# songlab-cal/CherryML

Measured on AMD Instinct MI355X. Metric: cherry-pairs/sec (whole node) per EM iter, higher is better.
Workload: dtype f64

## Files before the change

### cherryml_amd/csrc/eigh_planned.hip.h

```cpp
#pragma once
#include "jacobi_block.hip.h"
#include "large_bank.hip.h"

enum {
  EC_STALL = 0,
  EC_FINAL = 1,
  EC_NSWEEP = 2,
  EC_MODE = 3,
  EC_SQ = 4,
  EC_ERR = 5,
  EC_ARRIVE = 6,
  EC_MASKED = 7,
  EC_SC = 8,
  EC_BANDS = 9,
  EC_SIGMA = 10,
  EC_TBSTALE = 11,
  EC_SKIP = 12,
  EC_REC = 16,
  EC_MAXREC = 12,
  EC_JSTATE = 64,
  EC_T0 = 80,
  EC_TSWEEP = 81,
  EC_TEND = 93,
  EC_NSTAMP = 95,
  EC_STAMPS = 96,
#ifdef CB_EIGH_STAMPS
  EC_WORDS = 96 + 96
#else
  EC_WORDS = 96
#endif
};
#ifdef CB_EIGH_STAMPS
__device__ __forceinline__ void lge_stamp(unsigned long long *ctl, int id) {
  if (blockIdx.x == 0 && blockIdx.y == 0 && threadIdx.x == 0) {
    const unsigned long long i = atomicAdd(ctl + EC_NSTAMP, 1ull);
    if (i < 96ull) ctl[EC_STAMPS + i] = ((unsigned long long)__builtin_amdgcn_s_memrealtime() << 8) | (unsigned long long)id;
  }
}
#define LGE_STAMP(ctl, id) lge_stamp(const_cast<unsigned long long *>(ctl), id)
#else

#define LGE_STAMP(ctl, id) ((void)0)
#endif
#define EC_NONE 0xFFFFFFFFull
#ifdef CB_PLAIN_WORDS
typedef const unsigned long long *lge_const_words;
#else
typedef const __attribute__((address_space(4))) unsigned long long *lge_const_words;
#endif

struct GramArgs {
  int LD, band, slot;
  int cap;
  int nsq;
  const double *G;
  double *X, *Xf;
  double *Gm, *dg;
  int so;
  unsigned long long *acc;
  unsigned long long *ctl;
  double trigger;
};

#define LGE_ACC_NT 32
#define LGE_ACC_COS 64
#define LGE_ACC_WORDS 128
#define LGE_ACC_UNIT 4503599627370496.0
__device__ __forceinline__ unsigned long long lge_fix(double x) {
  return x > 0.0 ? (unsigned long long)(fmin(x, 16.0) * LGE_ACC_UNIT) + 1ull : 0ull;
}

struct DecArgs {
  int on = 0;
  int cap = 0, nsq = 0, so = 0;
  double trigger = 0.0;
  const unsigned long long *acc = nullptr;
};

__device__ __forceinline__ double lge_lim(int order) {
  return order == 2 ? 1e-5 : order == 4 ? 2e-3 : order == 8 ? 0.06 : 0.5;
}

__global__ __launch_bounds__(512, 6) void lge_gram(GramArgs a) {
  __shared__ double sRed[8][256];
  __shared__ double sDg[2][32][16];
  __shared__ double sD[2][16];
  __shared__ double sStat[3][4];
  const unsigned long long *ctl = a.ctl;
  LGE_STAMP(ctl, 4);
  {
    lge_const_words cw = (lge_const_words)ctl;
    const unsigned long long w_stall = cw[EC_STALL], w_final = cw[EC_FINAL];
    if (w_stall != 0ull || (unsigned long long)a.slot > w_final) return;
  }
  const int LD = a.LD, nt = LD / 16;
  const int tm = blockIdx.x / nt, tn = blockIdx.x - tm * nt;
  const int m0 = tm * 16, n0 = tn * 16;
  const int wave = threadIdx.x >> 6, lane = threadIdx.x & 63, lo = lane & 15, hi = lane >> 4;
  const double *rowA = a.G + (size_t)(m0 + lo) * LD + 4 * hi, *rowB = a.G + (size_t)(n0 + lo) * LD + 4 * hi;
  d4 acc0 = {0.0, 0.0, 0.0, 0.0}, acc1 = acc0;
  double da = 0.0, db = 0.0;
  const int nchunks = LD / 16;
  for (int j0 = wave; j0 < nchunks; j0 += 32) {
    d4 av[4], bv[4];
#pragma unroll
    for (int u = 0; u < 4; ++u) {
      const int j = min(j0 + 8 * u, nchunks - 1);
      av[u] = *reinterpret_cast<const d4 *>(rowA + 16 * j);
      bv[u] = *reinterpret_cast<const d4 *>(rowB + 16 * j);
    }
#pragma unroll
    for (int u = 0; u < 4; ++u) {
      if (j0 + 8 * u < nchunks) {
        acc0 = mfma_f64(av[u][0], bv[u][0], acc0);
        acc1 = mfma_f64(av[u][1], bv[u][1], acc1);
        acc0 = mfma_f64(av[u][2], bv[u][2], acc0);
        acc1 = mfma_f64(av[u][3], bv[u][3], acc1);
        da += (av[u][0] * av[u][0] + av[u][1] * av[u][1]) + (av[u][2] * av[u][2] + av[u][3] * av[u][3]);
        db += (bv[u][0] * bv[u][0] + bv[u][1] * bv[u][1]) + (bv[u][2] * bv[u][2] + bv[u][3] * bv[u][3]);
      }
    }
  }
  const d4 acc = acc0 + acc1;
#pragma unroll
  for (int r = 0; r < 4; ++r) sRed[wave][r * 64 + lane] = acc[r];
  sDg[0][wave * 4 + hi][lo] = da;
  sDg[1][wave * 4 + hi][lo] = db;
  __syncthreads();
  if (threadIdx.x < 32) {
    const int w = threadIdx.x >> 4, c = threadIdx.x & 15;
    double s0 = 0.0, s1 = 0.0, s2 = 0.0, s3 = 0.0;
#pragma unroll
    for (int p = 0; p < 32; p += 4) {
      s0 += sDg[w][p][c];
      s1 += sDg[w][p + 1][c];
      s2 += sDg[w][p + 2][c];
      s3 += sDg[w][p + 3][c];
    }
    sD[w][c] = (s0 + s1) + (s2 + s3);
  }
  __syncthreads();
  double mc2 = 0.0;
  if (threadIdx.x < 256) {
    const int t = threadIdx.x, r = t >> 6, l = t & 63;
    const int ri = (l >> 4) + 4 * r, ci = l & 15;
    const int row = m0 + ri, col = n0 + ci;
    double g = 0.0;
#pragma unroll
    for (int w = 0; w < 8; ++w) g += sRed[w][t];
    const double gii = sD[0][ri], gjj = sD[1][ci];
    double x = 0.0;
    const double g2 = g * g, ab = gii * gjj;
    if (!(g2 == g2) || !(ab == ab)) mc2 = INFINITY;
    if (row != col && g2 > ab * (CB_JAC_SKIP * CB_JAC_SKIP)) {
      mc2 = fmax(mc2, g2 * fast_rcp(ab));
      const double d = gjj - gii;
      x = d != 0.0 ? 0.5 * atan(2.0 * g * fast_rcp(d)) : (g > 0.0 ? 0.78539816339744831 : -0.78539816339744831);
    }
    const int bd = row / JB_W - col / JB_W;
    const bool far = bd > a.band || -bd > a.band;
    a.X[(size_t)row * LD + col] = x;
    a.Xf[(size_t)row * LD + col] = far ? x : 0.0;
    if (a.so) {
      a.Gm[(size_t)row * LD + col] = g;
      if (row == col) a.dg[row] = gii;
    }
    double rs = fabs(x), rsf = far ? fabs(x) : 0.0;
#pragma unroll
    for (int m = 1; m < 16; m <<= 1) {
      rs += __shfl_xor(rs, m);
      rsf += __shfl_xor(rsf, m);
      mc2 = fmax(mc2, __shfl_xor(mc2, m));
    }
#pragma unroll
    for (int m = 16; m < 64; m <<= 1) {
      rs = fmax(rs, __shfl_xor(rs, m));
      rsf = fmax(rsf, __shfl_xor(rsf, m));
      mc2 = fmax(mc2, __shfl_xor(mc2, m));
    }
    if (l == 0) {
      sStat[0][r] = rs;
      sStat[1][r] = rsf;
      sStat[2][r] = mc2;
    }
  }
  __syncthreads();
  if (threadIdx.x < 3) {
    const int k = threadIdx.x;
    const double v = fmax(fmax(sStat[k][0], sStat[k][1]), fmax(sStat[k][2], sStat[k][3]));
    if (k < 2) atomicAdd(a.acc + k * LGE_ACC_NT + tm, lge_fix(v));
    else atomicMax(a.acc + LGE_ACC_COS + 16 * (blockIdx.x & 3), dbl_bits(v));
  }
}

struct LgeDecision {
  unsigned long long mode, sq, sc_bits;
};
struct LgeAcc {
  unsigned long long w = 0ull, c2 = 0ull;
};
__device__ __forceinline__ LgeAcc lge_acc_request(const DecArgs &d) {
  LgeAcc q;
  if (d.on) {
    q.w = d.acc[threadIdx.x & 63];
    lge_const_words ar = (lge_const_words)d.acc;
#pragma unroll
    for (int i = 0; i < 4; ++i) {
      const unsigned long long c = ar[LGE_ACC_COS + 16 * i];
      q.c2 = c > q.c2 ? c : q.c2;
    }
  }
  return q;
}
__device__ __forceinline__ double lge_uniform(double v, int lane) {
  return __hiloint2double(__builtin_amdgcn_readlane(__double2hiint(v), lane), __builtin_amdgcn_readlane(__double2loint(v), lane));
}
__device__ __forceinline__ LgeDecision lge_decide_here(int slot, const DecArgs &d, const LgeAcc &q, unsigned long long *ctl,
                                                       unsigned long long nsweep) {
  double v = (double)q.w * (1.0 / LGE_ACC_UNIT);
#pragma unroll
  for (int m = 1; m < 32; m <<= 1) v = fmax(v, __shfl_xor(v, m));
  const double rowsum = lge_uniform(v, 0), rowsum_far = lge_uniform(v, 32);
  double c2;
  memcpy(&c2, &q.c2, 8);
  LgeDecision o{0ull, 0ull, 0x3FF0000000000000ull};
  const bool bad = q.c2 >= 0x7FF0000000000000ull;
  bool masked = false, fin = false;
  if (!bad) {
    masked = c2 > d.trigger * d.trigger || rowsum > 1.0;
    const double rsu = masked ? rowsum_far : rowsum;
    const bool so = d.so != 0 && !masked && c2 > 1e-16 && rowsum <= 0.3;
    const double r2 = rowsum * rowsum;
    fin = !masked && (c2 <= 1e-16 || (so && c2 * r2 * r2 <= 4e-28));
    int order = rsu <= lge_lim(2) ? 2 : rsu <= lge_lim(4) ? 4 : rsu <= lge_lim(8) ? 8 : 12;
    if (order > d.cap) order = d.cap;
    const double lim = lge_lim(order);
    double sc = 1.0;
    while (rsu * sc > lim) {
      sc *= 0.5;
      ++o.sq;
    }
    unsigned long long damped = 0ull;
    if (o.sq > (unsigned long long)d.nsq) {
// ... 45 lines not shown
    double r = -lam[k] * Ut[(size_t)k * LD + i];
    for (int j = 0; j < LD; ++j) r = fma(A[(size_t)i * LD + j], Ut[(size_t)k * LD + j], r);
    m = fmax(m, fabs(r));
    if (!(r == r)) m = INFINITY;
  }
  m = wave_max(m);
  if ((threadIdx.x & 63) == 0) atomicMax(ctl + 92, dbl_bits(m));
}
#endif
#ifdef CB_NANCHECK
__global__ void lge_orthcheck(int LD, const double *R, unsigned long long slot, unsigned long long *ctl) {
  lge_const_words cw = (lge_const_words)ctl;
  if (cw[EC_STALL] != 0ull || slot > cw[EC_FINAL] || !(cw[EC_MODE] >> 16)) return;
  const int k = blockIdx.x;
  double m = 0.0;
  for (int j = threadIdx.x; j < LD; j += blockDim.x) {
    double d = j == k ? -1.0 : 0.0;
    for (int i = 0; i < LD; ++i) d = fma(R[(size_t)i * LD + k], R[(size_t)i * LD + j], d);
    m = fmax(m, fabs(d));
    if (!(d == d)) m = INFINITY;
  }
  m = wave_max(m);
  if ((threadIdx.x & 63) == 0) {
    const unsigned long long old = atomicMax(ctl + 91, dbl_bits(m));
    if (dbl_bits(m) > old) ctl[90] = slot;
  }
}
#endif
#ifdef CB_NANCHECK
__global__ void lge_nancheck(int LD, const double *buf, unsigned long long tag, unsigned long long *ctl) {
  const size_t i = (size_t)blockIdx.x * blockDim.x + threadIdx.x;
  if (i >= (size_t)LD * LD) return;
  const double v = buf[i];
  if (!(v - v == 0.0)) atomicCAS(ctl + 94, 0ull, tag);
}
#endif

enum { EG_P2 = 0, EG_P34, EG_T1, EG_RP, EG_SQ, EG_GR, EG_R4 };

struct EgArgs {
  int LD, slot, kind, q;
  int cap;
  int early;
  const unsigned long long *ctl;
  const double *X, *Xf;
  double *P2, *P4;
  double *B0, *B1, *B2;
  double *T;
  double *R[2], *Rt[2];
  double *Rfin;
  const double *Gin;
  double *Gout;
  DecArgs dec;
  unsigned long long *zacc;
};


__device__ __forceinline__ double lge_ld(const double *base, int s, int LD, int c0, unsigned lane_bytes) {
  const __amdgpu_buffer_rsrc_t rs = __builtin_amdgcn_make_buffer_rsrc(const_cast<double *>(base), 0, 0x7fffffff, 0x00027000);
  return __builtin_bit_cast(double, __builtin_amdgcn_raw_buffer_load_b64(rs, (int)lane_bytes, (int)((unsigned)(4 * s * LD + c0) * 8u), 0));
}

__device__ __forceinline__ double lge_fold8(double (*sRed)[256], d4 acc, int wave, int lane, int et) {
  if (wave >= 4) {
#pragma unroll
    for (int r = 0; r < 4; ++r) sRed[wave - 4][r * 64 + lane] = acc[r];
  }
  __syncthreads();
  if (wave < 4) {
#pragma unroll
    for (int r = 0; r < 4; ++r) acc[r] += sRed[wave][r * 64 + lane];
  }
  __syncthreads();
  if (wave < 4) {
#pragma unroll
    for (int r = 0; r < 4; ++r) sRed[wave][r * 64 + lane] = acc[r];
  }
  __syncthreads();
  return (sRed[0][et] + sRed[1][et]) + (sRed[2][et] + sRed[3][et]);
}

#define LGE_UU 13
template <int KIND>
__global__ __launch_bounds__(512) void lge_gemm(EgArgs a) {
  __shared__ double sRed[4][256];
  const unsigned long long *ctl = a.ctl;
  LGE_STAMP(ctl, 10 + KIND);
  const int LD = a.LD, nt = LD / 16;
  const int tm = blockIdx.x / nt, tn = blockIdx.x - tm * nt;
  const int m0 = tm * 16, n0 = tn * 16;
  const int wave = __builtin_amdgcn_readfirstlane(threadIdx.x >> 6), lane = threadIdx.x & 63, lo = lane & 15, hi = lane >> 4;
  const int nsteps = LD / 4;
  const unsigned loff = (unsigned)(hi * LD + lo) * 8u;
  const int et = threadIdx.x & 255, er = et >> 6, el = et & 63;
  const int row = m0 + (el >> 4) + 4 * er, col = n0 + (el & 15);
  const size_t idx = (size_t)row * LD + col;
  const bool ep = threadIdx.x < 256;
  const double *Ap = nullptr, *Bp = nullptr, *Ep = nullptr;
  if (KIND == EG_T1) { Ap = a.P4; Bp = a.B2; Ep = a.B1; }
  if (KIND == EG_RP) { Ap = a.P4; Bp = a.T; Ep = a.B0; }
  if (KIND == EG_SQ) { Ap = a.Rt[a.q & 1]; Bp = a.R[a.q & 1]; }
  if (KIND == EG_GR) { Ap = a.Rfin; Bp = a.Gin; }
  if (KIND == EG_R4) { Ap = a.P2; Bp = a.B0; Ep = a.P2; }
  double av[LGE_UU], bv[LGE_UU], e1 = 0.0, ex = 0.0;
  const bool early = KIND != EG_P2 && a.early != 0;
  if (early) {
#pragma unroll
    for (int u = 0; u < LGE_UU; ++u) {
      const int sk = min(wave + 8 * u, nsteps - 1);
      av[u] = lge_ld(Ap, sk, LD, m0, loff);
      bv[u] = lge_ld(Bp, sk, LD, n0, loff);
    }
    if (Ep && ep) e1 = Ep[idx];
  }
  LgeAcc accq;
  if (KIND == EG_P2) accq = lge_acc_request(a.dec);
  lge_const_words cw = (lge_const_words)ctl;
  const unsigned long long w_stall = cw[EC_STALL], w_final = cw[EC_FINAL], w_nsw = cw[EC_NSWEEP];
  unsigned long long mode = cw[EC_MODE], w_sq = cw[EC_SQ], w_sc = cw[EC_SC];
  if (w_stall != 0ull || (unsigned long long)a.slot > w_final) return;
  if (KIND == EG_P2 && a.dec.on) {
    const LgeDecision dd = lge_decide_here(a.slot, a.dec, accq, const_cast<unsigned long long *>(ctl), w_nsw);
    mode = dd.mode;
    w_sq = dd.sq;
    w_sc = dd.sc_bits;
  }
  if (!(mode >> 16)) return;
  if (KIND == EG_GR && a.zacc && blockIdx.x == 0 && threadIdx.x < LGE_ACC_WORDS)
    a.zacc[threadIdx.x] = 0ull;
  const int order = (int)(mode & 255ull);
  const bool masked = (mode & (256ull | 1024ull)) != 0ull;
  const int sq = (int)w_sq;
  double sc;
  memcpy(&sc, &w_sc, 8);
  const double *Xu = masked ? a.Xf : a.X;
  if (KIND == EG_R4 && order != 4) return;
  if (KIND == EG_T1 && order != 12) return;
  if (KIND == EG_RP && order < 8) return;
  if (KIND == EG_SQ && a.q >= sq) return;
  if (!early) {
    const double *pa = KIND == EG_P2 ? Xu : Ap, *pb = KIND == EG_P2 ? Xu : Bp;
#pragma unroll
    for (int u = 0; u < LGE_UU; ++u) {
      const int sk = min(wave + 8 * u, nsteps - 1);
      av[u] = lge_ld(pa, sk, LD, m0, loff);
      bv[u] = lge_ld(pb, sk, LD, n0, loff);
    }
    if (KIND != EG_P2 && Ep && ep) e1 = Ep[idx];
  }
  if ((KIND == EG_P2 || KIND == EG_R4) && ep) ex = Xu[idx];
  d4 acc = {0.0, 0.0, 0.0, 0.0};
#pragma unroll
  for (int u = 0; u < LGE_UU; ++u)
    if (wave + 8 * u < nsteps) acc = mfma_f64(av[u], bv[u], acc);
  for (int s0 = wave + 8 * LGE_UU; s0 < nsteps; s0 += 8 * LGE_UU) {
    const double *pa = KIND == EG_P2 ? Xu : Ap, *pb = KIND == EG_P2 ? Xu : Bp;
#pragma unroll
    for (int u = 0; u < LGE_UU; ++u) {
      const int sk = min(s0 + 8 * u, nsteps - 1);
      av[u] = lge_ld(pa, sk, LD, m0, loff);
      bv[u] = lge_ld(pb, sk, LD, n0, loff);
    }
#pragma unroll
    for (int u = 0; u < LGE_UU; ++u)
      if (s0 + 8 * u < nsteps) acc = mfma_f64(av[u], bv[u], acc);
  }
  const double v = lge_fold8(sRed, acc, wave, lane, et);
  if (!ep) return;
  const double edl = row == col ? 1.0 : 0.0, s2 = sc * sc;
  if (KIND == EG_P2) {
    if (order == 2) {
      a.Rfin[idx] = fma(-0.5 * s2, v, fma(sc, ex, edl));
    } else {
      a.P2[idx] = v;
      if (a.cap == 4) a.B0[idx] = fma(-s2 * (1.0 / 24.0), v, (sc * (1.0 / 6.0)) * ex);
    }
  } else if (KIND == EG_R4) {
    a.Rfin[idx] = fma(-s2, v, fma(-0.5 * s2, e1, fma(sc, ex, edl)));
  } else if (KIND == EG_T1) {
    a.T[idx] = fma(s2 * s2, v, e1);
  } else if (KIND == EG_RP) {
    const double o = fma(s2 * s2, v, e1);
    if (sq == 0) a.Rfin[idx] = o;
    else {
      a.R[0][idx] = o;
      a.Rt[0][(size_t)col * LD + row] = o;
    }
  } else if (KIND == EG_SQ) {
    if (a.q == sq - 1) a.Rfin[idx] = v;
    else {
      a.R[(a.q + 1) & 1][idx] = v;
      a.Rt[(a.q + 1) & 1][(size_t)col * LD + row] = v;
    }
  } else {
    a.Gout[idx] = v;
  }
}

__global__ __launch_bounds__(512) void lge_p34(EgArgs a) {
  __shared__ double sRed[8][256];
  const unsigned long long *ctl = a.ctl;
  LGE_STAMP(ctl, 17);
  const int LD = a.LD, nt = LD / 16;
  const int tm = blockIdx.x / nt, tn = blockIdx.x - tm * nt;
  const int m0 = tm * 16, n0 = tn * 16;
  const int wave = __builtin_amdgcn_readfirstlane(threadIdx.x >> 6), lane = threadIdx.x & 63, lo = lane & 15, hi = lane >> 4;
  const int w4 = wave & 3;
  const bool fourth = wave >= 4;
  const int nsteps = LD / 4;
  const unsigned loff = (unsigned)(hi * LD + lo) * 8u;
  const int et = threadIdx.x & 255, er = et >> 6, el = et & 63;
  const int row = m0 + (el >> 4) + 4 * er, col = n0 + (el & 15);
  const size_t idx = (size_t)row * LD + col;
  const bool ep = threadIdx.x < 256;
  double av[LGE_UU], bv[LGE_UU], e2 = 0.0;
  const bool early = a.early != 0;
  if (early) {
#pragma unroll
    for (int u = 0; u < LGE_UU; ++u) {
      const int sk = min(w4 + 4 * u, nsteps - 1);
// ... 24 lines not shown
  } else if (!fourth) {
#pragma unroll
    for (int u = 0; u < LGE_UU; ++u) av[u] = lge_ld(Xu, min(w4 + 4 * u, nsteps - 1), LD, m0, loff);
  }
  double ex = 0.0;
  if (ep) ex = Xu[idx];
  d4 acc = {0.0, 0.0, 0.0, 0.0};
#pragma unroll
  for (int u = 0; u < LGE_UU; ++u)
    if (w4 + 4 * u < nsteps) acc = mfma_f64(av[u], bv[u], acc);
  for (int s0 = w4 + 4 * LGE_UU; s0 < nsteps; s0 += 4 * LGE_UU) {
#pragma unroll
    for (int u = 0; u < LGE_UU; ++u) {
      const int sk = min(s0 + 4 * u, nsteps - 1);
      av[u] = lge_ld(Ap, sk, LD, m0, loff);
      bv[u] = lge_ld(a.P2, sk, LD, n0, loff);
    }
#pragma unroll
    for (int u = 0; u < LGE_UU; ++u)
      if (s0 + 4 * u < nsteps) acc = mfma_f64(av[u], bv[u], acc);
  }
#pragma unroll
  for (int r = 0; r < 4; ++r) sRed[wave][r * 64 + lane] = acc[r];
  __syncthreads();
  if (!ep) return;
  const double p3 = (sRed[0][et] + sRed[1][et]) + (sRed[2][et] + sRed[3][et]);
  const double p4 = (sRed[4][et] + sRed[5][et]) + (sRed[6][et] + sRed[7][et]);
  const double dl = row == col ? 1.0 : 0.0;
  const double s2 = sc * sc;
  const double y1 = sc * ex, y2 = -s2 * e2, y3 = s2 * sc * p3, y4 = s2 * s2 * p4;
  const double b0 = dl + y1 + 0.5 * y2 + y3 * (1.0 / 6.0);
  if (order == 4) {
    a.Rfin[idx] = b0 + y4 * (1.0 / 24.0);
    return;
  }
  a.P4[idx] = p4;
  a.B0[idx] = b0;
  const double b1 = dl * (1.0 / 24.0) + y1 * (1.0 / 120.0) + y2 * (1.0 / 720.0) + y3 * (1.0 / 5040.0);
  if (order == 8) {
    a.T[idx] = b1 + y4 * (1.0 / 40320.0);
    return;
  }
  a.B1[idx] = b1;
  a.B2[idx] = dl * (1.0 / 40320.0) + y1 * (1.0 / 362880.0) + y2 * (1.0 / 3628800.0) + y3 * (1.0 / 39916800.0) + y4 * (1.0 / 479001600.0);
}

struct SoArgs {
  int LD, slot;
  const unsigned long long *ctl;
  const double *Gm, *dg, *X;
  double *Xs;
  int early;
  DecArgs dec;
};

__global__ __launch_bounds__(512) void lge_so(SoArgs a) {
  __shared__ double sRed[4][256];
  const unsigned long long *ctl = a.ctl;
  LGE_STAMP(ctl, 6);
  const int LD = a.LD, nt = LD / 16;
  const int tm = blockIdx.x / nt, tn = blockIdx.x - tm * nt;
  const int m0 = tm * 16, n0 = tn * 16;
  const int wave = threadIdx.x >> 6, lane = threadIdx.x & 63, lo = lane & 15, hi = lane >> 4;
  d4 accA = {0.0, 0.0, 0.0, 0.0}, accB = accA;
  const int nsteps = LD / 4;
  const double *Em = a.Gm + m0 + lo, *En = a.Gm + n0 + lo, *Xm = a.X + m0 + lo, *Xn = a.X + n0 + lo;
  double e1[7], x1[7], x2[7], e2[7];
  auto issue = [&](int s0) {
#pragma unroll
    for (int u = 0; u < 7; ++u) {
      const int s = min(s0 + 8 * u, nsteps - 1);
      const int k = 4 * s + hi;
      const size_t krow = (size_t)k * LD;
      e1[u] = k == m0 + lo ? 0.0 : Em[krow];
      x1[u] = Xn[krow];
      x2[u] = Xm[krow];
      e2[u] = k == n0 + lo ? 0.0 : En[krow];
    }
  };
  if (a.early) issue(wave);
  const LgeAcc accq = lge_acc_request(a.dec);
  lge_const_words cw = (lge_const_words)ctl;
  const unsigned long long w_stall = cw[EC_STALL], w_final = cw[EC_FINAL], w_nsw = cw[EC_NSWEEP];
  unsigned long long w_mode = cw[EC_MODE];
  if (w_stall != 0ull || (unsigned long long)a.slot > w_final) return;
  if (a.dec.on) w_mode = lge_decide_here(a.slot, a.dec, accq, const_cast<unsigned long long *>(ctl), w_nsw).mode;
  if (!(w_mode & 1024ull)) return;
  for (int s0 = wave; s0 < nsteps; s0 += 7 * 8) {
    if (!(a.early && s0 == wave)) issue(s0);
#pragma unroll
    for (int u = 0; u < 7; ++u)
      if (s0 + 8 * u < nsteps) {
        accA = mfma_f64(e1[u], x1[u], accA);
        accB = mfma_f64(x2[u], e2[u], accB);
      }
  }
  d4 acc = accA + accB;
  if (wave >= 4) {
#pragma unroll
    for (int r = 0; r < 4; ++r) sRed[wave - 4][r * 64 + lane] = acc[r];
  }
  __syncthreads();
  if (wave < 4) {
#pragma unroll
    for (int r = 0; r < 4; ++r) acc[r] += sRed[wave][r * 64 + lane];
  }
  __syncthreads();
  if (wave < 4) {
#pragma unroll
    for (int r = 0; r < 4; ++r) sRed[wave][r * 64 + lane] = acc[r];
  }
  __syncthreads();
  if (threadIdx.x >= 256) return;
  const int t = threadIdx.x, r = t >> 6, l = t & 63;
  const int row = m0 + (l >> 4) + 4 * r, col = n0 + (l & 15);
  const double v = (sRed[0][t] + sRed[1][t]) + (sRed[2][t] + sRed[3][t]);
  const size_t idx = (size_t)row * LD + col;
  const double x1v = a.X[idx];
  const double d = a.dg[col] - a.dg[row];
  double xs = x1v;
  if (row != col && x1v != 0.0 && d != 0.0) xs = 0.5 * atan(2.0 * (a.Gm[idx] + 0.5 * v) * fast_rcp(d));
  a.Xs[idx] = xs;
}

__device__ void lge_reset_words(unsigned long long *ctl, unsigned long long *acc) {
  if (threadIdx.x < EC_WORDS)
    ctl[threadIdx.x] = threadIdx.x == EC_FINAL ? EC_NONE : threadIdx.x == EC_T0 ? (unsigned long long)__builtin_amdgcn_s_memrealtime() : 0ull;
  if (threadIdx.x < 2 * LGE_ACC_WORDS) acc[threadIdx.x] = 0ull;
}
__global__ void lge_begin(int LD, const double *A, double *sigma, unsigned long long *ctl, unsigned long long *acc) {
  __shared__ double s[256];
  lge_reset_words(ctl, acc);
  double m = 0.0;
  for (int i = threadIdx.x; i < LD; i += 256) m = fmax(m, fabs(A[(size_t)i * LD + i]));
  s[threadIdx.x] = m;
  __syncthreads();
  for (int st = 128; st >= 1; st >>= 1) {
    if ((int)threadIdx.x < st) s[threadIdx.x] = fmax(s[threadIdx.x], s[threadIdx.x + st]);
    __syncthreads();
  }
  if (threadIdx.x == 0) *sigma = s[0] > 0.0 ? s[0] : 1.0;
}

__global__ __launch_bounds__(512) void lge_plain(int LD, const double *Aop, const double *Bop, const double *Sub, const double *sigma,
                                                 double *out, const unsigned long long *skip) {
  __shared__ double sRed[4][256];
  const int nt = LD / 16;
  const int tm = blockIdx.x / nt, tn = blockIdx.x - tm * nt;
  const int m0 = tm * 16, n0 = tn * 16;
  const int wave = __builtin_amdgcn_readfirstlane(threadIdx.x >> 6), lane = threadIdx.x & 63, lo = lane & 15, hi = lane >> 4;
  const int nsteps = LD / 4;
  const unsigned loff = (unsigned)(hi * LD + lo) * 8u;
  const int et = threadIdx.x & 255, er = et >> 6, el = et & 63;
  const int row = m0 + (el >> 4) + 4 * er, col = n0 + (el & 15);
  const size_t idx = (size_t)row * LD + col;
  double av[LGE_UU], bv[LGE_UU];
#pragma unroll
  for (int u = 0; u < LGE_UU; ++u) {
    const int sk = min(wave + 8 * u, nsteps - 1);
    av[u] = lge_ld(Aop, sk, LD, m0, loff);
    bv[u] = lge_ld(Bop, sk, LD, n0, loff);
  }
  const double e1 = (Sub && threadIdx.x < 256) ? Sub[idx] : 0.0;
  const double sg = sigma ? *sigma : 0.0;
  if (skip && *(lge_const_words)skip != 0ull) return;
  d4 acc = {0.0, 0.0, 0.0, 0.0};
#pragma unroll
  for (int u = 0; u < LGE_UU; ++u)
    if (wave + 8 * u < nsteps) acc = mfma_f64(av[u], bv[u], acc);
// ... 122 lines not shown
```

### cherryml_amd/csrc/eigh_planned_host.hip.h

```cpp
#pragma once

struct EighRecord {
  bool stall = false;
  int err = 0, nsweep = 0, final_slot = -1;
  double sigma = 0.0;
  bool tb_stale = false;
  struct {
    double c, rs, rsf;
    int order, sq, slot;
    bool masked, damped;
  } sweep[EC_MAXREC];
};

#ifndef CB_PLANNED_BAND
#define CB_PLANNED_BAND 1
#endif
#ifndef CB_LEAD_INNER
#define CB_LEAD_INNER 2
#endif
static const int kPlannedBand = CB_PLANNED_BAND;

static void eigh_plan_default(EighPlan &p, int extra = 0) {
  p = EighPlan{};
  p.lead_band = 1;
// ... 62 lines not shown
    memset(q, 0, 2 * (EC_WORDS + 16) * sizeof(unsigned long long));
    h->epin = static_cast<unsigned long long *>(q);
  }
  const int RS = LD + ((2 - LD % 32 + 32) % 32);
  const size_t lds = (size_t)(16 * RS + 3 * 16 * 17 + JB_WAVES * 256) * sizeof(double);
  if (hipFuncSetAttribute(reinterpret_cast<const void *>(lgj_round), hipFuncAttributeMaxDynamicSharedMemorySize, (int)lds) != hipSuccess)
    return false;
  if (hipMemsetAsync(ctl, 0, EC_WORDS * sizeof(unsigned long long), h->stream) != hipSuccess) return false;
  h->ectl = ctl;
  h->planned_unavailable = false;
  return true;
}

#ifdef CB_NANCHECK
#define NANCHECK(buf, tag) hipLaunchKernelGGL(lge_nancheck, dim3((unsigned)((LL + 255) / 256)), dim3(256), 0, h->stream, LD, buf, (unsigned long long)(tag), ctl)
#else
#define NANCHECK(buf, tag) ((void)0)
#endif
static int enqueue_planned_solve(cb_bank *h, const EighPlan &p, unsigned long long seq, int first_slot = 0, double tb_rho_max = 0.0,
                                 const TbTableArgs &tbt = TbTableArgs{}) {
  const int LD = h->LD, nt = LD / 16, nb = LD / JB_W;
  const size_t LL = (size_t)LD * LD;
  unsigned long long *ctl = h->ectl;
  unsigned long long *eacc = reinterpret_cast<unsigned long long *>(h->epart);
  double *Gb[2] = {h->Gc, h->Gc2};
  double *X = h->gx, *Xf = h->gx + LL, *P2 = h->gx + 2 * LL, *P3 = h->gx + 3 * LL, *P4 = h->gx + 4 * LL, *B0 = h->gx + 5 * LL,
         *B1 = h->gx + 6 * LL, *B2 = h->gx + 7 * LL, *T = h->gx + 8 * LL, *R0 = h->gx + 9 * LL, *R0t = h->gx + 10 * LL,
         *R1 = h->gx + 11 * LL, *R1t = h->gx + 6 * LL,
         *Rfin = h->gx + 3 * LL;
  const int RS = LD + ((2 - LD % 32 + 32) % 32);
  const size_t lds = (size_t)(16 * RS + 3 * 16 * 17 + JB_WAVES * 256) * sizeof(double);
  if (first_slot > 0) {
    hipLaunchKernelGGL(lge_resume, dim3(1), dim3(64), 0, h->stream, ctl);
  } else {
    if (!h->begin_folded) hipLaunchKernelGGL(lge_begin, dim3(1), dim3(256), 0, h->stream, LD, h->A, h->sigma, ctl, eacc);
    NANCHECK(h->U, 1);
    NANCHECK(h->A, 2);
    hipLaunchKernelGGL(lge_plain, dim3((unsigned)(nt * nt)), dim3(512), 0, h->stream, LD, h->U, h->A, h->Vc, h->sigma, Gb[0], nullptr);
  }
  unsigned long long *jstate = ctl + EC_JSTATE;
  int shift = 0;
  auto band_pass = [&](double *G, const unsigned long long *must_nonzero) {
    for (int w = 0; w < 2; ++w)
      hipLaunchKernelGGL(lgj_round, dim3(nb / 2), dim3(JB_THREADS), lds, h->stream, LD, ((shift + w) & 1) && nb > 2 ? -2 : -1,
                         must_nonzero ? 1 : CB_LEAD_INNER, G,
                         jstate, ctl + EC_STALL, must_nonzero);
    for (int k = 2; k <= kPlannedBand && k < nb; ++k)
      for (int par = 0; par < 2; ++par)
        hipLaunchKernelGGL(lgj_round, dim3((unsigned)(((nb + 2 * k - 1) / (2 * k)) * k)), dim3(JB_THREADS), lds, h->stream, LD,
                           -(10 + 2 * (k - 2) + par), 0, G, jstate, ctl + EC_STALL, must_nonzero);
    ++shift;
  };
  if (p.lead_band) band_pass(Gb[first_slot & 1], nullptr);
  const dim3 tiles((unsigned)(nt * nt));
  for (int i = 0; i < p.nslots; ++i) {
    const EighSlot &q = p.slot[i];
    const int s = first_slot + i;
    double *Gin = Gb[s & 1], *Gout = Gb[(s + 1) & 1];
    unsigned long long *acc = eacc + (size_t)(s & 1) * LGE_ACC_WORDS;
    GramArgs ga{LD, kPlannedBand, s, q.cap, q.cap == 12 ? q.nsq : 0, Gin, X, Xf, P3, h->epart + (size_t)2 * LGE_ACC_WORDS,
                q.so, acc, ctl, 3e-4};
    NANCHECK(Gin, 1000 + s * 100 + 1);
    hipLaunchKernelGGL(lge_gram, tiles, dim3(512), 0, h->stream, ga);
    NANCHECK(X, 1000 + s * 100 + 2);
    DecArgs dec;
    dec.on = 1; dec.cap = ga.cap; dec.nsq = ga.nsq; dec.so = q.so; dec.acc = acc; dec.trigger = ga.trigger;
#ifdef CB_DECIDE_KERNEL
    hipLaunchKernelGGL(lge_decide_k, dim3(1), dim3(64), 0, h->stream, s, dec, ctl);
    dec.on = 0;
#endif
    if (q.so) {
      SoArgs so{LD, s, ctl, ga.Gm, ga.dg, X, Xf, q.expect_run && i >= 1, dec};
#ifdef CB_NO_EARLY
      so.early = 0;
#endif
      hipLaunchKernelGGL(lge_so, tiles, dim3(512), 0, h->stream, so);
      NANCHECK(Xf, 1000 + s * 100 + 3);
    }
    EgArgs e{};
    if (!q.so) e.dec = dec;
    e.zacc = acc;
    e.LD = LD; e.slot = s; e.cap = q.cap; e.ctl = ctl; e.X = X; e.Xf = Xf; e.P2 = P2; e.P4 = P4; e.B0 = B0; e.B1 = B1; e.B2 = B2; e.T = T;
    e.R[0] = R0; e.R[1] = R1; e.Rt[0] = R0t; e.Rt[1] = R1t; e.Rfin = Rfin; e.Gin = Gin; e.Gout = Gout;
    auto gemm = [&](int kind, int qq = 0) {
      EgArgs c = e;
      c.kind = kind;
      c.q = qq;
      const int xo = q.expect_order;
      c.early = !q.expect_run ? 0 : kind == EG_P34 ? xo >= 4 : kind == EG_T1 ? xo == 12 : kind == EG_RP ? xo >= 8 :
                kind == EG_SQ ? qq < q.expect_sq : kind == EG_R4 ? xo == 4 : 1;
#ifdef CB_NO_EARLY
      c.early = 0;
#endif
      switch (kind) {
        case EG_P2: hipLaunchKernelGGL(lge_gemm<EG_P2>, tiles, dim3(512), 0, h->stream, c); break;
        case EG_P34: hipLaunchKernelGGL(lge_p34, tiles, dim3(512), 0, h->stream, c); break;
        case EG_T1: hipLaunchKernelGGL(lge_gemm<EG_T1>, tiles, dim3(512), 0, h->stream, c); break;
        case EG_RP: hipLaunchKernelGGL(lge_gemm<EG_RP>, tiles, dim3(512), 0, h->stream, c); break;
        case EG_SQ: hipLaunchKernelGGL(lge_gemm<EG_SQ>, tiles, dim3(512), 0, h->stream, c); break;
        case EG_R4: hipLaunchKernelGGL(lge_gemm<EG_R4>, tiles, dim3(512), 0, h->stream, c); break;
        default: hipLaunchKernelGGL(lge_gemm<EG_GR>, tiles, dim3(512), 0, h->stream, c); break;
      }
    };
    gemm(EG_P2);
    if (q.cap == 12) {
      gemm(EG_P34);
      gemm(EG_T1);
      gemm(EG_RP);
      for (int k = 0; k < q.nsq; ++k) gemm(EG_SQ, k);
    } else if (q.cap == 4) {
      gemm(EG_R4);
    }
    NANCHECK(Rfin, 1000 + s * 100 + 4);
#ifdef CB_NANCHECK
    hipLaunchKernelGGL(lge_orthcheck, dim3((unsigned)LD), dim3(256), 0, h->stream, LD, Rfin, (unsigned long long)s, ctl);
#endif
    gemm(EG_GR);
    NANCHECK(Gout, 1000 + s * 100 + 5);
    if (q.band_after) band_pass(Gout, ctl + EC_MASKED);
  }
  volatile unsigned long long *pin = h->epin + (size_t)(seq & 1ull) * (EC_WORDS + 16);
  hipLaunchKernelGGL(lge_norms, dim3((LD + 3) / 4), dim3(256), 0, h->stream, LD, Gb[0], Gb[1], h->X, ctl, pin, seq, h->sigma, tb_rho_max);
  LAUNCH_STOP(stop_event(h, EV_EIGH), lge_finish, dim3((LD + 3) / 4 + 1), dim3(256), 0, h->stream, LD, Gb[0], Gb[1], h->X, h->sigma, h->lam, h->U, h->Vc,
                     ctl, tbt, pin, seq);
#ifdef CB_NANCHECK
  hipLaunchKernelGGL(lge_residual, dim3((unsigned)LD), dim3(256), 0, h->stream, LD, h->A, h->Vc, h->lam, ctl);
#endif
  HIP_TRY(hipGetLastError());
  return CB_OK;
}

static int eigh_planned_record(cb_bank *h, unsigned long long seq, EighRecord &r) {
  volatile unsigned long long *pin = h->epin + (size_t)(seq & 1ull) * (EC_WORDS + 16);
  const auto t0 = std::chrono::steady_clock::now();
  bool got = false;
  for (unsigned it = 0;; ++it) {
    if (pin[EC_WORDS] == seq) {
      got = true;
      break;
    }
    if (it == 0) ++h->record_spins;
#if defined(__x86_64__)
    __builtin_ia32_pause();
#endif
    if ((it & 4095u) == 4095u && std::chrono::duration<double, std::milli>(std::chrono::steady_clock::now() - t0).count() > 200.0) break;
  }
  if (!got) {
    HIP_TRY(hipStreamSynchronize(h->stream));
// ... 70 lines not shown
```

### cherryml_amd/csrc/handle_host.hip.h

```cpp
#pragma once
#include <hip/hip_ext.h>
#include <future>
struct EighSlot {
  int cap = 12;
  int nsq = 0;
  int band_after = 0;
  int so = 0;
  int expect_run = 1, expect_order = 12, expect_sq = 2;
};
struct EighPlan {
  int lead_band = 1;
  int nslots = 0;
  EighSlot slot[EC_MAXREC];
};
struct cb_bank {
  int dev = 0, S = 0, L = 0, B = 0;
  int B_cap = 0;
  hipStream_t xstream[3] = {};
  hipEvent_t ev_fork = nullptr, ev_join[3] = {};
  int tr_epochs = 0;
  uint64_t tr_sig = 0;
  int last_form = 0;
  double tr_pow_b1 = 1.0, tr_pow_b2 = 1.0;
  int dtype = CB_F64;
  int LD = 0;
  bool large = false;
  hipStream_t own_stream = nullptr, stream = nullptr;
  std::vector<void *> allocs;
  std::vector<double> n_host;
  double *t = nullptr;
  double *Ct = nullptr;
  double *n_dev = nullptr;
  double *inv_n = nullptr;
  double *ones = nullptr;
  double *Cq = nullptr;
  int nq = 0;
  double *dirsum = nullptr;
  double *dirsum_g = nullptr;
  int Bl = 0;
  double *t_live = nullptr;
  int *nlive = nullptr;
  std::vector<int> nlive_host;
  double *Q = nullptr, *pi = nullptr, *loss = nullptr, *dQ = nullptr;
  int *status = nullptr;
  double *Gc2 = nullptr, *gx = nullptr;
  int last_light = 0;
  void *comm = nullptr;
  int (*allreduce)(const void *, void *, size_t, int, int, void *, hipStream_t) = nullptr;
  double *inv_n_global = nullptr;
  std::vector<double> n_global;
  bool expm_only = false;
  bool per_bucket_products = false;
  bool sym_counts = false;
  int spec_sweeps = 0;
  double *A = nullptr, *dsq = nullptr, *Gc = nullptr, *Vc = nullptr, *U = nullptr, *lam = nullptr,
         *sigma = nullptr, *F = nullptr, *E = nullptr, *H = nullptr, *Gt = nullptr, *T = nullptr,
         *Mt_part = nullptr, *Mt = nullptr, *X = nullptr, *loss_part = nullptr;
  float *Ct32 = nullptr, *Gt32 = nullptr, *T32 = nullptr, *Uf = nullptr, *Utf = nullptr, *Af = nullptr, *Ff = nullptr;
  unsigned long long *off_bits = nullptr;
  unsigned long long *poll = nullptr;
  unsigned long long poll_seq = 0;
  unsigned long long *ectl = nullptr, *epin = nullptr;
  double *epart = nullptr;
  bool begin_folded = false;
  double *sigma_home = nullptr;
  double *sigma2 = nullptr;
  unsigned long long eseq = 0;
  bool planned_unavailable = false;
  int planned_solves = 0, planned_stalls = 0;
  long long record_spins = 0;
  std::vector<double> epoch_seconds;
  EighPlan eplan;
  int k3_chunk = 0, k3_nchunks = 0;
  double *Yk = nullptr, *Lk = nullptr;
  double phi_delta = 0.0;
  unsigned int *bank_queue = nullptr;
  unsigned char *bank_args = nullptr;
  int bank_slots = 0;
  int bank_claims = 0;
  bool bank_fused = false;
  int bank_kg = 1;
  bool bank_accum = false;
  CbTimeBasisHost tb;
  int tb_set = 0;
  double *tb_Ls[2] = {}, *tb_Lg[2] = {}, *tb_tf[2] = {}, *tb_tg[2] = {};
  std::future<CbTimeBasisHost> tb_next;
  bool tb_next_pending = false;
  int tb_next_epoch = 0;
  size_t tb_ew_lds[4] = {0, 0, 0, 0};
  int tb_builds = 0, tb_stale_epochs = 0;
  bool tb_failed = false;
  bool tb_block = false;
  bool bank_tb = false;
  int last_sweeps = 0;
  double *gn_scratch = nullptr, *gn_partial = nullptr;
  int gn_nw = 0;
  struct {
    double *Qn = nullptr, *QT = nullptr, *colsum = nullptr, *alpha = nullptr, *R = nullptr, *RT = nullptr, *E = nullptr,
           *ET = nullptr, *G = nullptr, *GT = nullptr, *Xbar = nullptr, *lpart = nullptr;
    int *nsq = nullptr;
    int cap_slots = 0;
  } gl;
  std::vector<double> t_host, t_live_host;
  bool have_prev = false;
  double *ws_ptr[16] = {};
  size_t ws_cap[16] = {};
  char *pin = nullptr;
  size_t pin_cap = 0, pin_off = 0;
  bool profile = false;
  int profile_every = 1;
  bool profile_now = false;
  hipEvent_t ev[CB_T_COUNT + 1] = {};
  bool ev_rec[CB_T_COUNT + 1] = {};
  double t_sum[CB_T_COUNT] = {};
  int t_calls = 0;
  bool t_pending = false;
  hipEvent_t ev2[CB_T_COUNT + 1] = {};
  bool ev_rec2[CB_T_COUNT + 1] = {};
  bool t_pending2 = false;
};

// ... 102 lines not shown
```

### cherryml_amd/csrc/train_host.hip.h

```cpp
#pragma once
template <int NW>
static int launch_train_nw(cb_bank *h, const TrainArgs &a) {
  static_assert(NW == 4, "25 .. 32 states: the four-wave form only (see the kernels' launch bounds)");
  const size_t lds = (SmallLds<NW>::TOTAL + 72) * sizeof(double);
  if (h->S <= 24) return fail(CB_EINVAL, "internal: %d states dispatched to the one-kernel trainer", h->S);
  auto kern = small_train_kernel<2, 8, NW>;
  HIP_TRY(hipFuncSetAttribute(reinterpret_cast<const void *>(kern), hipFuncAttributeMaxDynamicSharedMemorySize, (int)lds));
  hipLaunchKernelGGL(kern, dim3(h->L), dim3(NW * 64), lds, h->stream, a);
  HIP_TRY(hipGetLastError());
  return CB_OK;
}

__global__ void tr_stamp(double *out) { *out = (double)__builtin_amdgcn_s_memrealtime(); }

static void set_epoch_seconds(cb_bank *h, const char *ticks, int E, double t_first_s) {
  h->epoch_seconds.assign((size_t)std::max(E, 0), 0.0);
  if (!ticks || E <= 0) return;
  std::vector<double> tk((size_t)E + 1);
  memcpy(tk.data(), ticks, ((size_t)E + 1) * sizeof(double));
  for (int e = 0; e < E; ++e) h->epoch_seconds[e] = t_first_s + (tk[e] - tk[E]) * 1e-8;
}

static int run_fused_training_large(cb_bank *h, double *pi_param, double *up_param, const double *mask, int E,
                                    double lr, int do_adam, int flags, double *loss_curve, double *Q_best,
// ... 52 lines not shown
    return fail(CB_ENOMEM, "fused training: device allocation failed");
  }
  if (dbg) fprintf(stderr, "[cherrybank] large trainer: workspaces ready after %.2f ms\n", now() - t_enter);
  int rc = CB_OK;
#define TRYH(expr) \
  if (rc == CB_OK && (expr) != hipSuccess) rc = fail(CB_EHIP, "%s failed", #expr)
  {
    const size_t up_bytes = (S + nup + SS + 64) * sizeof(double);
    const size_t down_bytes = (S + nup + 2 * (size_t)E + 16 + (2 + (size_t)(d_Qp ? n_pow2 : 0)) * SS + 64) * sizeof(double);
    if (!pin_reserve(h, std::max(up_bytes, down_bytes) + 1024)) {
      release();
      return fail(CB_ENOMEM, "fused training: pinned staging allocation failed");
    }
  }
  if (!resume) {
    TRYH(h2d_staged(h, d_pi, pi_param, S * sizeof(double)));
    TRYH(h2d_staged(h, d_up, up_param, nup * sizeof(double)));
    TRYH(hipMemsetAsync(d_mom, 0, nmom * sizeof(double), h->stream));
    TRYH(hipMemsetAsync(d_Qb, 0, SS * sizeof(double), h->stream));
    TRYH(hipMemsetAsync(d_Ql, 0, SS * sizeof(double), h->stream));
  }
  if (mask && !resume) TRYH(h2d_staged(h, d_mask, mask, SS * sizeof(double)));
  const double init_state[2] = {INFINITY, INFINITY};
  LargeTrain a{};
  a.S = S; a.LD = LD; a.do_adam = do_adam; a.n_pow2 = d_Qp ? n_pow2 : 0;
  a.epoch0 = e0;
  a.p_pi = d_pi; a.p_up = d_up;
  a.m_pi = d_mom; a.v_pi = d_mom + S; a.m_up = d_mom + 2 * (size_t)S; a.v_up = a.m_up + nup;
  a.mask = d_mask; a.lr = lr; a.beta1 = 0.9; a.beta2 = 0.999; a.eps = 1e-8;
  a.pi = d_vec; a.gd = d_vec + LD; a.state = d_vec + LD + S;
  a.dsq = h->dsq; a.A = h->A; a.G = h->Mt; a.loss = h->loss;
  a.dirsum = h->comm ? h->dirsum_g : h->dirsum;
  a.inv_n = (flags & CB_NORMALIZE) ? 1.0 / (h->comm ? h->n_global[0] : h->n_host[0]) : 1.0;
  a.loss_curve = d_loss; a.time_curve = d_time; a.Q_last = d_Ql; a.Q_best = d_Qb; a.Q_pow2 = d_Qp;
  if (dbg) fprintf(stderr, "[cherrybank] large trainer: copies enqueued after %.2f ms\n", now() - t_enter);
  if (!resume) TRYH(h2d_staged(h, a.state, init_state, sizeof init_state));
  TRYH(hipStreamSynchronize(h->stream));
  if (dbg) fprintf(stderr, "[cherrybank] large trainer: synced after %.2f ms\n", now() - t_enter);
  if (h->profile) fold_pending(h);
  if (dbg) fprintf(stderr, "[cherrybank] large trainer: parameters uploaded after %.2f ms\n", now() - t_enter);
  double pow_b1 = resume ? h->tr_pow_b1 : 1.0, pow_b2 = resume ? h->tr_pow_b2 : 1.0;
  if (!h->sigma2) {
    if (dev_alloc(h, &h->sigma2, 2) != CB_OK) {
      release();
      return CB_ENOMEM;
    }
  }
  if (!h->sigma_home) h->sigma_home = h->sigma;
  TRYH(hipMemsetAsync(h->sigma2, 0, 2 * sizeof(double), h->stream));
  h->last_form = 4000;
  h->tr_epochs = 0;
  const int fault_epoch = cb_test_hook("CB_FAULT_INJECT") ? atoi(cb_test_hook("CB_FAULT_INJECT")) : -1000;
  const bool planned = !cb_test_hook("CB_EIGH_HOST") && !cb_test_hook("CB_NO_HYBRID") && LD % 16 == 0 && LD / JB_W >= 8 && eigh_planned_setup(h);
  EighPlan &plan = h->eplan;
  if (!resume) eigh_plan_default(plan);
  if (!resume) {
    tb_drop_next(h);
    h->tb = CbTimeBasisHost{};
    h->tb_failed = false;
  }
  const int short_plans = cb_test_hook("CB_EIGH_SHORT_PLAN") ? std::max(1, atoi(cb_test_hook("CB_EIGH_SHORT_PLAN"))) : 0;
  auto shorten = [&]() {
    if (!short_plans) return;
    plan.nslots = 1;
    if (short_plans >= 2) plan.slot[0] = EighSlot{2, 0, plan.slot[0].band_after, 0};
  };
  shorten();
  const double trace_slow = getenv("CB_TRACE_SLOW") ? atof(getenv("CB_TRACE_SLOW")) : 0.0;
  const double t_first_s = (now() - t_enter) * 1e-3;
  hipLaunchKernelGGL(tr_stamp, dim3(1), dim3(1), 0, h->stream, d_time + E);
  for (int e = 0; e < E && rc == CB_OK; ++e) {
    const double te0 = trace_slow > 0.0 ? now() : 0.0;
    double te_fold = 0.0, te_enq = 0.0, te_rec = 0.0;
    h->profile_now = h->profile && (e0 + e) % h->profile_every == 0;
    if (h->profile_now) {
      swap_event_sets(h);
      fold_pending(h);
    }
    if (trace_slow > 0.0) te_fold = now();
    clear_marks(h);
    const bool use_plan = planned && h->have_prev && e0 + e >= 3;
    {
      const int par = (e0 + e) & 1;
      h->sigma = h->sigma2 + par;
      a.sig_cur = reinterpret_cast<unsigned long long *>(h->sigma2 + par);
      a.sig_next = reinterpret_cast<unsigned long long *>(h->sigma2 + (par ^ 1));
      a.ectl = use_plan ? h->ectl : nullptr;
      a.eacc = use_plan ? reinterpret_cast<unsigned long long *>(h->epart) : nullptr;
      h->begin_folded = use_plan;
    }
    LAUNCH_STOP(stop_event(h, EV_START), lt_build, dim3(LD), dim3(256), 0, h->stream, a, e0 + e);
    rc = large_eval(h, flags & CB_NORMALIZE, h->loss, h->Mt, true, nullptr, false, use_plan ? &plan : nullptr);
    h->begin_folded = false;
    if (trace_slow > 0.0) te_enq = now();
    if (rc == CB_OK && use_plan) {
      EighRecord rec;
      rc = eigh_planned_record(h, h->eseq, rec);
      ++h->planned_solves;
      if (rc == CB_OK && rec.err == 2) rc = fail(CB_ENUMERIC, "eigensolver: non-finite input");
      int slots_done = plan.nslots;
      for (int attempt = 0; rc == CB_OK && rec.stall && attempt < 3; ++attempt) {
        ++h->planned_stalls;
        EighPlan more;
        eigh_plan_continue(rec, more);
        clear_marks(h);
        mark(h, EV_START);
// ... 347 lines not shown
```

Baseline: 1.546 billion.

## Compute only upper-triangle tiles of symmetric Gram/P2/SO products and mirror

The Gram, second-order and P2 GEMM kernels now launch one block per upper-triangular 16x16 tile pair instead of every tile. Each off-diagonal block writes both its tile and the transposed mirror, using the upper 256 threads that were previously idle in the epilogue. A folded index mapping pairs row q with row nt-1-q so blocks stay balanced. This roughly halves the MFMA work and reads for these symmetric products. The cost is extra epilogue stores, per-row accumulator atomics for both rows, and a lower occupancy hint on lge_gram. An env hook restores full tiling.

```diff
diff --git a/cherryml_amd/csrc/eigh_planned.hip.h b/cherryml_amd/csrc/eigh_planned.hip.h
--- a/cherryml_amd/csrc/eigh_planned.hip.h
+++ b/cherryml_amd/csrc/eigh_planned.hip.h
@@ -60,6 +60,7 @@
   unsigned long long *acc;
   unsigned long long *ctl;
   double trigger;
+  int pair;
 };
 
 #define LGE_ACC_NT 32
@@ -81,11 +82,25 @@
   return order == 2 ? 1e-5 : order == 4 ? 2e-3 : order == 8 ? 0.06 : 0.5;
 }
 
-__global__ __launch_bounds__(512, 6) void lge_gram(GramArgs a) {
+__device__ __forceinline__ void lge_tile(int b, int nt, bool pair, int &tm, int &tn) {
+  const int dv = pair ? nt + 1 : nt;
+  const int q = b / dv, c = b - q * dv;
+  tm = q;
+  tn = c;
+  if (pair) {
+    if (c < nt - q) tn = q + c;
+    else {
+      tm = nt - 1 - q;
+      tn = tm + (c - (nt - q));
+    }
+  }
+}
+
+__global__ __launch_bounds__(512, 4) void lge_gram(GramArgs a) {
   __shared__ double sRed[8][256];
   __shared__ double sDg[2][32][16];
   __shared__ double sD[2][16];
-  __shared__ double sStat[3][4];
+  __shared__ double sStat[2][3][4];
   const unsigned long long *ctl = a.ctl;
   LGE_STAMP(ctl, 4);
   {
@@ -94,7 +109,8 @@
     if (w_stall != 0ull || (unsigned long long)a.slot > w_final) return;
   }
   const int LD = a.LD, nt = LD / 16;
-  const int tm = blockIdx.x / nt, tn = blockIdx.x - tm * nt;
+  int tm, tn;
+  lge_tile((int)blockIdx.x, nt, a.pair != 0, tm, tn);
   const int m0 = tm * 16, n0 = tn * 16;
   const int wave = threadIdx.x >> 6, lane = threadIdx.x & 63, lo = lane & 15, hi = lane >> 4;
   const double *rowA = a.G + (size_t)(m0 + lo) * LD + 4 * hi, *rowB = a.G + (size_t)(n0 + lo) * LD + 4 * hi;
@@ -140,15 +156,17 @@
     sD[w][c] = (s0 + s1) + (s2 + s3);
   }
   __syncthreads();
+  const bool mir = threadIdx.x >= 256, two = a.pair != 0 && tm != tn;
   double mc2 = 0.0;
-  if (threadIdx.x < 256) {
-    const int t = threadIdx.x, r = t >> 6, l = t & 63;
+  if (!mir || two) {
+    const int t = threadIdx.x & 255, r = t >> 6, l = t & 63;
     const int ri = (l >> 4) + 4 * r, ci = l & 15;
-    const int row = m0 + ri, col = n0 + ci;
+    const int row = (mir ? n0 : m0) + ri, col = (mir ? m0 : n0) + ci;
+    const int ts = mir ? 16 * ci + ri : t;
     double g = 0.0;
 #pragma unroll
-    for (int w = 0; w < 8; ++w) g += sRed[w][t];
-    const double gii = sD[0][ri], gjj = sD[1][ci];
+    for (int w = 0; w < 8; ++w) g += sRed[w][ts];
+    const double gii = sD[mir ? 1 : 0][ri], gjj = sD[mir ? 0 : 1][ci];
     double x = 0.0;
     const double g2 = g * g, ab = gii * gjj;
     if (!(g2 == g2) || !(ab == ab)) mc2 = INFINITY;
@@ -179,16 +197,16 @@
       mc2 = fmax(mc2, __shfl_xor(mc2, m));
     }
     if (l == 0) {
-      sStat[0][r] = rs;
-      sStat[1][r] = rsf;
-      sStat[2][r] = mc2;
-    }
-  }
-  __syncthreads();
-  if (threadIdx.x < 3) {
-    const int k = threadIdx.x;
-    const double v = fmax(fmax(sStat[k][0], sStat[k][1]), fmax(sStat[k][2], sStat[k][3]));
-    if (k < 2) atomicAdd(a.acc + k * LGE_ACC_NT + tm, lge_fix(v));
+      sStat[mir][0][r] = rs;
+      sStat[mir][1][r] = rsf;
+      sStat[mir][2][r] = mc2;
+    }
+  }
+  __syncthreads();
+  if (threadIdx.x < (two ? 5 : 3)) {
+    const int k = threadIdx.x, h = k >= 3, kk = k - 3 * h;
+    const double v = fmax(fmax(sStat[h][kk][0], sStat[h][kk][1]), fmax(sStat[h][kk][2], sStat[h][kk][3]));
+    if (kk < 2) atomicAdd(a.acc + kk * LGE_ACC_NT + (h ? tn : tm), lge_fix(v));
     else atomicMax(a.acc + LGE_ACC_COS + 16 * (blockIdx.x & 3), dbl_bits(v));
   }
 }
@@ -340,6 +358,7 @@
   const double *Gin;
   double *Gout;
   DecArgs dec;
+  int pair;
   unsigned long long *zacc;
 };
 
@@ -375,15 +394,18 @@
   const unsigned long long *ctl = a.ctl;
   LGE_STAMP(ctl, 10 + KIND);
   const int LD = a.LD, nt = LD / 16;
-  const int tm = blockIdx.x / nt, tn = blockIdx.x - tm * nt;
+  int tm, tn;
+  lge_tile((int)blockIdx.x, nt, KIND == EG_P2 && a.pair != 0, tm, tn);
   const int m0 = tm * 16, n0 = tn * 16;
   const int wave = __builtin_amdgcn_readfirstlane(threadIdx.x >> 6), lane = threadIdx.x & 63, lo = lane & 15, hi = lane >> 4;
   const int nsteps = LD / 4;
   const unsigned loff = (unsigned)(hi * LD + lo) * 8u;
-  const int et = threadIdx.x & 255, er = et >> 6, el = et & 63;
-  const int row = m0 + (el >> 4) + 4 * er, col = n0 + (el & 15);
+  const bool mir = KIND == EG_P2 && a.pair != 0 && tm != tn && threadIdx.x >= 256;
+  const int et = threadIdx.x & 255, eri = et >> 4, eci = et & 15;
+  const int es = mir ? 16 * eci + eri : et;
+  const int row = (mir ? n0 : m0) + eri, col = (mir ? m0 : n0) + eci;
   const size_t idx = (size_t)row * LD + col;
-  const bool ep = threadIdx.x < 256;
+  const bool ep = threadIdx.x < 256 || mir;
   const double *Ap = nullptr, *Bp = nullptr, *Ep = nullptr;
   if (KIND == EG_T1) { Ap = a.P4; Bp = a.B2; Ep = a.B1; }
   if (KIND == EG_RP) { Ap = a.P4; Bp = a.T; Ep = a.B0; }
@@ -453,7 +475,7 @@
     for (int u = 0; u < LGE_UU; ++u)
       if (s0 + 8 * u < nsteps) acc = mfma_f64(av[u], bv[u], acc);
   }
-  const double v = lge_fold8(sRed, acc, wave, lane, et);
+  const double v = lge_fold8(sRed, acc, wave, lane, es);
   if (!ep) return;
   const double edl = row == col ? 1.0 : 0.0, s2 = sc * sc;
   if (KIND == EG_P2) {
@@ -584,6 +606,7 @@
   double *Xs;
   int early;
   DecArgs dec;
+  int pair;
 };
 
 __global__ __launch_bounds__(512) void lge_so(SoArgs a) {
@@ -591,7 +614,8 @@
   const unsigned long long *ctl = a.ctl;
   LGE_STAMP(ctl, 6);
   const int LD = a.LD, nt = LD / 16;
-  const int tm = blockIdx.x / nt, tn = blockIdx.x - tm * nt;
+  int tm, tn;
+  lge_tile((int)blockIdx.x, nt, a.pair != 0, tm, tn);
   const int m0 = tm * 16, n0 = tn * 16;
   const int wave = threadIdx.x >> 6, lane = threadIdx.x & 63, lo = lane & 15, hi = lane >> 4;
   d4 accA = {0.0, 0.0, 0.0, 0.0}, accB = accA;
@@ -643,10 +667,12 @@
     for (int r = 0; r < 4; ++r) sRed[wave][r * 64 + lane] = acc[r];
   }
   __syncthreads();
-  if (threadIdx.x >= 256) return;
-  const int t = threadIdx.x, r = t >> 6, l = t & 63;
-  const int row = m0 + (l >> 4) + 4 * r, col = n0 + (l & 15);
-  const double v = (sRed[0][t] + sRed[1][t]) + (sRed[2][t] + sRed[3][t]);
+  const bool mir = threadIdx.x >= 256;
+  if (mir && !(a.pair != 0 && tm != tn)) return;
+  const int t = threadIdx.x & 255, ri = t >> 4, ci = t & 15;
+  const int ts = mir ? 16 * ci + ri : t;
+  const int row = (mir ? n0 : m0) + ri, col = (mir ? m0 : n0) + ci;
+  const double v = (sRed[0][ts] + sRed[1][ts]) + (sRed[2][ts] + sRed[3][ts]);
   const size_t idx = (size_t)row * LD + col;
   const double x1v = a.X[idx];
   const double d = a.dg[col] - a.dg[row];
diff --git a/cherryml_amd/csrc/eigh_planned_host.hip.h b/cherryml_amd/csrc/eigh_planned_host.hip.h
--- a/cherryml_amd/csrc/eigh_planned_host.hip.h
+++ b/cherryml_amd/csrc/eigh_planned_host.hip.h
@@ -138,16 +138,17 @@
     ++shift;
   };
   if (p.lead_band) band_pass(Gb[first_slot & 1], nullptr);
-  const dim3 tiles((unsigned)(nt * nt));
+  const int pair = h->eigh_full_tiles ? 0 : 1;
+  const dim3 tiles((unsigned)(nt * nt)), mtiles((unsigned)(pair ? nt * (nt + 1) / 2 : nt * nt));
   for (int i = 0; i < p.nslots; ++i) {
     const EighSlot &q = p.slot[i];
     const int s = first_slot + i;
     double *Gin = Gb[s & 1], *Gout = Gb[(s + 1) & 1];
     unsigned long long *acc = eacc + (size_t)(s & 1) * LGE_ACC_WORDS;
     GramArgs ga{LD, kPlannedBand, s, q.cap, q.cap == 12 ? q.nsq : 0, Gin, X, Xf, P3, h->epart + (size_t)2 * LGE_ACC_WORDS,
-                q.so, acc, ctl, 3e-4};
+                q.so, acc, ctl, 3e-4, pair};
     NANCHECK(Gin, 1000 + s * 100 + 1);
-    hipLaunchKernelGGL(lge_gram, tiles, dim3(512), 0, h->stream, ga);
+    hipLaunchKernelGGL(lge_gram, mtiles, dim3(512), 0, h->stream, ga);
     NANCHECK(X, 1000 + s * 100 + 2);
     DecArgs dec;
     dec.on = 1; dec.cap = ga.cap; dec.nsq = ga.nsq; dec.so = q.so; dec.acc = acc; dec.trigger = ga.trigger;
@@ -156,16 +157,17 @@
     dec.on = 0;
 #endif
     if (q.so) {
-      SoArgs so{LD, s, ctl, ga.Gm, ga.dg, X, Xf, q.expect_run && i >= 1, dec};
+      SoArgs so{LD, s, ctl, ga.Gm, ga.dg, X, Xf, q.expect_run && i >= 1, dec, pair};
 #ifdef CB_NO_EARLY
       so.early = 0;
 #endif
-      hipLaunchKernelGGL(lge_so, tiles, dim3(512), 0, h->stream, so);
+      hipLaunchKernelGGL(lge_so, mtiles, dim3(512), 0, h->stream, so);
       NANCHECK(Xf, 1000 + s * 100 + 3);
     }
     EgArgs e{};
     if (!q.so) e.dec = dec;
     e.zacc = acc;
+    e.pair = pair;
     e.LD = LD; e.slot = s; e.cap = q.cap; e.ctl = ctl; e.X = X; e.Xf = Xf; e.P2 = P2; e.P4 = P4; e.B0 = B0; e.B1 = B1; e.B2 = B2; e.T = T;
     e.R[0] = R0; e.R[1] = R1; e.Rt[0] = R0t; e.Rt[1] = R1t; e.Rfin = Rfin; e.Gin = Gin; e.Gout = Gout;
     auto gemm = [&](int kind, int qq = 0) {
@@ -179,7 +181,7 @@
       c.early = 0;
 #endif
       switch (kind) {
-        case EG_P2: hipLaunchKernelGGL(lge_gemm<EG_P2>, tiles, dim3(512), 0, h->stream, c); break;
+        case EG_P2: hipLaunchKernelGGL(lge_gemm<EG_P2>, mtiles, dim3(512), 0, h->stream, c); break;
         case EG_P34: hipLaunchKernelGGL(lge_p34, tiles, dim3(512), 0, h->stream, c); break;
         case EG_T1: hipLaunchKernelGGL(lge_gemm<EG_T1>, tiles, dim3(512), 0, h->stream, c); break;
         case EG_RP: hipLaunchKernelGGL(lge_gemm<EG_RP>, tiles, dim3(512), 0, h->stream, c); break;
diff --git a/cherryml_amd/csrc/handle_host.hip.h b/cherryml_amd/csrc/handle_host.hip.h
--- a/cherryml_amd/csrc/handle_host.hip.h
+++ b/cherryml_amd/csrc/handle_host.hip.h
@@ -67,6 +67,7 @@
   double *sigma2 = nullptr;
   unsigned long long eseq = 0;
   bool planned_unavailable = false;
+  bool eigh_full_tiles = false;
   int planned_solves = 0, planned_stalls = 0;
   long long record_spins = 0;
   std::vector<double> epoch_seconds;
diff --git a/cherryml_amd/csrc/train_host.hip.h b/cherryml_amd/csrc/train_host.hip.h
--- a/cherryml_amd/csrc/train_host.hip.h
+++ b/cherryml_amd/csrc/train_host.hip.h
@@ -128,6 +128,10 @@
   h->tr_epochs = 0;
   const int fault_epoch = cb_test_hook("CB_FAULT_INJECT") ? atoi(cb_test_hook("CB_FAULT_INJECT")) : -1000;
   const bool planned = !cb_test_hook("CB_EIGH_HOST") && !cb_test_hook("CB_NO_HYBRID") && LD % 16 == 0 && LD / JB_W >= 8 && eigh_planned_setup(h);
+  {
+    const char *ft = cb_test_hook("CB_EIGH_FULL_TILES");
+    h->eigh_full_tiles = ft && ft[0] != '0' && ft[0] != 0;
+  }
   EighPlan &plan = h->eplan;
   if (!resume) eigh_plan_default(plan);
   if (!resume) {
```

Measured after the change: 1.571 billion, median of 4. About the same (+1.6%).
